# Stefo01/multigrid_prj

Measured on AMD Instinct MI355X. Metric: V-cycles/sec (3D Poisson 513^3 V(2,2)) + finest-grid smoother GB/s vs HBM roofline, higher is better.
Workload: dtype f64; 1 GPU; 3D Poisson 513^3 nodes (nominal 512^3), 6-level V(2,2), jacobi omega=6/7, full-weighting, coarse 17^3 iterated to rel. residual 0.1, f64; parallelism=single GPU, first_gathered_level=6

## Files before the change

__graft_entry__.py:

```python
import os
import subprocess
import sys

ROOT = os.path.dirname(os.path.abspath(__file__))
if ROOT not in sys.path:
    sys.path.insert(0, ROOT)


def build() -> None:
    from multigrid_prj_amd import build as b
    from multigrid_prj_amd import capi
    path = b.build(force=True, verbose=True)
    lib = capi.load(build_if_missing=False)
    missing = [s for s in capi.EXPORTS if not hasattr(lib, s)]
    assert not missing, missing
    subprocess.run(["make", "-C", os.path.join(ROOT, "oracle"), "-B", "_build/liboracle.so"], check=True)
    subprocess.run(["make", "-C", os.path.join(ROOT, "oracle"), "ref"], check=True)
    b.build_cli()
    build_pairbench()
    print("built", path)


def build_pairbench() -> str:
    from concurrent.futures import ThreadPoolExecutor
    csrc = os.path.join(ROOT, "multigrid_prj_amd", "csrc")
    out = os.path.join(ROOT, "tools", "pairbench")
    srcs = [os.path.join(ROOT, "tools", "pairbench.hip")] + [os.path.join(csrc, f) for f in
            ("mg_jacobi_fast.hip", "mg_pair_wide.hip", "mg_rr_wide.hip", "mg_transfer_fast.hip")]
    deps = srcs + [os.path.join(csrc, f) for f in ("mg_kernels.h", "mg_geom.h", "mg_device.h", "mg_switches.h", "mg_switches.def")]
    if os.path.exists(out) and all(os.path.getmtime(out) >= os.path.getmtime(f) for f in deps):
        return out
    objdir = os.path.join(ROOT, "multigrid_prj_amd", "lib", "obj")
    os.makedirs(objdir, exist_ok=True)
    flags = ["-O3", "--offload-arch=gfx950", "-ffp-contract=off", "-std=c++17", "-I" + os.path.join(ROOT, "include")]

    def cc(src):
        obj = os.path.join(objdir, "pb_" + os.path.basename(src) + ".o")
        subprocess.run(["/opt/rocm/bin/hipcc", *flags, "-c", src, "-o", obj], check=True)
        return obj

    with ThreadPoolExecutor(max_workers=5) as ex:
        objs = list(ex.map(cc, srcs))
    subprocess.run(["/opt/rocm/bin/hipcc", "--offload-arch=gfx950", *objs, "-o", out], check=True)
    return out


def smoke() -> None:
    import numpy as np
    from multigrid_prj_amd import capi
    from oracle import pyoracle as po

    assert capi.device_count() > 0, "smoke() needs a GPU"
    kw = dict(dim=2, n=65, levels=3, alpha=1.0, length=10.0, smoother=capi.SMOOTH_JACOBI)
    b = po.fill_rhs_2d(65, 10.0, 1)
    with capi.Solver(capi.make_desc(**kw)) as s:
        s.set_rhs(b)
        hist, _ = s.solve(1e-11, 50)
        o = po.Solver(po.make_desc(**kw)); o.set_rhs(b)
        href, _ = o.solve(1e-11, 50)
        assert len(hist) == len(href), (len(hist), len(href))
        np.testing.assert_allclose(hist, href, rtol=2e-3)
        np.testing.assert_allclose(s.get_solution(), o.get_solution(), rtol=1e-7, atol=1e-9)
    kw = dict(dim=3, n=65, levels=3, length=1.0, alpha=1.0, cycle=capi.CYCLE_V, smoother=capi.SMOOTH_JACOBI,
              omega=6 / 7, nu_pre=2, nu_post=2, coarse_mode=capi.COARSE_FIXED, coarse_maxit=20, outer_pre_gs=0)
    b = po.fill_rhs_3d(65, 1.0, 1.0, 1)
    with capi.Solver(capi.make_desc(**kw)) as s:
        s.set_rhs(b); s.cycle(); s.cycle()
        o = po.Solver(po.make_desc(**kw)); o.set_rhs(b); o.cycle(); o.cycle()
        assert np.array_equal(s.get_solution(), o.get_solution())
    print("smoke ok: 2-D sawtooth history", hist[-1], "3-D V-cycle bit-exact")


if __name__ == "__main__":
    build() if (len(sys.argv) < 2 or sys.argv[1] == "build") else smoke()
```

multigrid_prj_amd/csrc/mg_pair_wide.hip:

```cpp
#include "mg_kernels.h"
#include "mg_device.h"

#include <algorithm>
#include <cmath>

namespace mg {
namespace {

__device__ __forceinline__ float lane_bcast(float v, int l) { return __int_as_float(__builtin_amdgcn_readlane(__float_as_int(v), l)); }
__device__ __forceinline__ double lane_bcast(double v, int l)
{
    const int lo = __builtin_amdgcn_readlane(__double2loint(v), l), hi = __builtin_amdgcn_readlane(__double2hiint(v), l);
    return __hiloint2double(hi, lo);
}

template <typename T, int TPR, int G, bool DAMPED, bool CORR, bool ZEROU, bool RB = false, bool NORM = false>
__global__ __launch_bounds__(TPR * G) void k_pairw(Geom g, Coef<T> c, T omega, const T *__restrict__ u_,
                                                   const T *__restrict__ rhs_, T *__restrict__ out_, int nby, int zc,
                                                   const T *__restrict__ coarse, Geom gc, int dup_planes,
                                                   double *__restrict__ partials)
{
    constexpr int V = Vec16<T>::n, CV = V / 2, NR = CV + 1;
    constexpr int R = 2, NROW = G * R, S = NROW - 2;
    constexpr int LP = TPR * V + 2 * V;
    typedef T vec __attribute__((ext_vector_type(V)));
    static_assert(G >= 2 && (TPR % 64) == 0, "row-wide wave teams, at least two groups");
    __shared__ __align__(16) T su[ZEROU ? 1 : 2][ZEROU ? 1 : NROW + 2][ZEROU ? V : LP];
    __shared__ __align__(16) T sv[2][NROW][LP];
    __shared__ double snorm[NORM ? TPR * G / 64 : 1];

    const int t = threadIdx.x, lane = t & 63;
    const int grp = __builtin_amdgcn_readfirstlane(t / TPR);
    const int xt = t - grp * TPR;
    const int x0 = V * xt;
    const bool tail = (xt == TPR - 1);
    const bool tailwave = (xt >> 6) == (TPR >> 6) - 1;
    const int i0 = grp * R;
    const bool lo_grp = (grp == 0), hi_grp = (grp == G - 1);
    double nsq = 0.;
    const long long per_copy = (long long)nby * g.nz, total = (dup_planes > 0 ? 2 : 1) * per_copy;
    const int nwg = (int)gridDim.x, wper = nwg >> 3;
    const int wi = xcd_block(blockIdx.x, wper);
    const int nbz = zc > 0 ? (g.nz + zc - 1) / zc : 0;
    const long long items = (dup_planes > 0 ? 2 : 1) * (long long)nby * nbz;
    long long w0 = zc > 0 ? wi : total * wi / nwg;
    const long long w1 = zc > 0 ? items : total * (wi + 1) / nwg;
    while (w0 < w1) {
    bool second;
    int by, z0, z1;
    if (zc > 0) {
        const long long per = (long long)nby * nbz;
        second = w0 >= per;
        const long long wr = w0 - (second ? per : 0);
        const int bz = (int)(wr / nby);
        by = (int)(wr - (long long)bz * nby);
        z0 = bz * zc; z1 = min(z0 + zc, g.nz);
        w0 += nwg;
    } else {
        second = w0 >= per_copy;
        const long long wr = w0 - (second ? per_copy : 0);
        by = (int)(wr / g.nz);
        z0 = (int)(wr - (long long)by * g.nz); z1 = (int)min((long long)g.nz, z0 + (w1 - w0));
        w0 += z1 - z0;
    }
    const long long dup_off = second ? (long long)dup_planes * g.plane : 0;
    const T *__restrict__ u = u_ + dup_off;
    const T *__restrict__ rhs = rhs_ + dup_off;
    T *__restrict__ out = out_ + dup_off;
    const int Y0 = by * S;

    long long urow[R];
    bool ybnd[R], outrow[R];
#pragma unroll
    for (int r = 0; r < R; r++) {
        const int y = Y0 + i0 + r, yc = min(y, g.ny - 1);
        ybnd[r] = (yc == 0) || (yc == g.ny - 1);
        urow[r] = (long long)yc * g.pitch;
        const int i = i0 + r;
        outrow[r] = (i >= 1 || by == 0) && (i <= NROW - 2) && (y < g.ny);
    }
    const int hy = lo_grp ? max(Y0 - 1, 0) : min(Y0 + NROW, g.ny - 1);
    const long long hrow = (long long)hy * g.pitch;
    const int hs = lo_grp ? 0 : NROW + 1;

    const int zhalo = (g.gnz != g.nz) ? 2 : 1;
    const int gzo = g.gz0 + (second ? dup_planes : 0), gzn = g.gnz;
    auto plane_of = [&](int p) { return (long long)min(max(p, -zhalo), g.nz - 1 + zhalo) * g.plane; };

    const T hf = (T)0.5;
    typedef T cwide __attribute__((ext_vector_type(NR <= 2 ? 2 : 4), aligned(CV * sizeof(T))));
    int crow[3] = {0, 0, 0};
    const int ic0 = CV * xt;
    if (CORR) {
        const int A = (Y0 + i0) >> 1;
        crow[0] = min(max(A - 1, 0), gc.ny - 1) * gc.pitch;
        crow[1] = min(A, gc.ny - 1) * gc.pitch;
        crow[2] = min(A + 1, gc.ny - 1) * gc.pitch;
    }
    auto cplane = [&](int P, int up1) {
        const int kc = ((gzo + P + up1) >> 1) - gc.gz0;
        return coarse + (long long)min(max(kc, -zhalo), gc.nz - 1 + zhalo) * gc.plane;
    };
    auto load_crow = [&](const T *base, int j, T (&d)[NR]) {
        const cwide w = *(const cwide *)((base + crow[j]) + ic0);
#pragma unroll
        for (int m = 0; m < NR; m++) d[m] = w[m];
    };
    auto raw = [&](int P, T (&Ra)[3][NR], T (&Rb)[3][NR]) {
        const T *c0 = cplane(P, 0);
        const bool odd = ((gzo + P) & 1) != 0;
        const T *c1 = cplane(P, 1);
#pragma unroll
        for (int j = 0; j < 3; j++) {
            if (j == 0 && !lo_grp) {
#pragma unroll
                for (int m = 0; m < NR; m++) { Ra[j][m] = 0; Rb[j][m] = 0; }
                continue;
            }
            load_crow(c0, j, Ra[j]);
            if (odd) load_crow(c1, j, Rb[j]);
            else {
#pragma unroll
                for (int m = 0; m < NR; m++) Rb[j][m] = 0;
            }
        }
    };
    auto zfin = [&](int P, const T (&Ra)[3][NR], const T (&Rb)[3][NR], T (&Z)[3][NR]) {
        const int gP = gzo + P;
        const bool in = (gP >= 0) && (gP < gzn), odd = (gP & 1) != 0;
#pragma unroll
        for (int j = 0; j < 3; j++) {
#pragma unroll
            for (int m = 0; m < NR; m++) {
                const T z = odd ? hf * (Ra[j][m] + Rb[j][m]) : Ra[j][m];
                Z[j][m] = in ? z : (T)0;
            }
        }
    };
    auto pe_vec = [&](const T (&Yr)[NR]) {
        vec w;
#pragma unroll
        for (int mm = 0; mm < CV; mm++) {
            w[2 * mm] = Yr[mm];
            w[2 * mm + 1] = hf * (Yr[mm] + Yr[mm + 1]);
        }
        return w;
    };
    auto add_vec = [&](vec a, vec w) {
        vec o;
#pragma unroll
        for (int e = 0; e < V; e++) o[e] = a[e] + w[e];
        return o;
    };
    auto correct = [&](const T (&Z)[3][NR], vec (&w)[R], T (&tl)[R], vec &h, T &htl, bool with_halo) {
        T Yodd[NR];
#pragma unroll
        for (int m = 0; m < NR; m++) Yodd[m] = hf * (Z[1][m] + Z[2][m]);
        w[0] = add_vec(w[0], pe_vec(Z[1]));
        w[1] = add_vec(w[1], pe_vec(Yodd));
        tl[0] = tl[0] + Z[1][CV];
        tl[1] = tl[1] + Yodd[CV];
        if (with_halo) {
            if (lo_grp) {
                T Yh[NR];
#pragma unroll
                for (int m = 0; m < NR; m++) Yh[m] = hf * (Z[0][m] + Z[1][m]);
                h = add_vec(h, pe_vec(Yh));
                htl = htl + Yh[CV];
            } else if (hi_grp) {
                h = add_vec(h, pe_vec(Z[2]));
                htl = htl + Z[2][CV];
            }
        }
    };

    auto update = [&](const vec &zm, const vec &cc, const vec &zp, const vec &ym, const vec &yp, T xm, T xp,
                      const vec &bb, bool rb) {
        T num[V], quo[V];
        vec res;
#pragma unroll
        for (int e = 0; e < V; e++) {
            const T left = (e == 0) ? xm : cc[e > 0 ? e - 1 : 0];
            const T right = (e == V - 1) ? xp : cc[e < V - 1 ? e + 1 : 0];
            T sum = 0;
            sum += c.cz * zm[e];
            sum += c.cy * ym[e];
            sum += c.cx * left;
            sum += c.cx * right;
            sum += c.cy * yp[e];
            sum += c.cz * zp[e];
            num[e] = bb[e] - sum;
        }
        if constexpr (sizeof(T) == 8) div_cd_n_wave<T, V>(num, quo, c);
        else div_cd_n<T, V>(num, quo, c);
#pragma unroll
        for (int e = 0; e < V; e++) {
            T jac = quo[e];
            if (DAMPED) jac = cc[e] + omega * (jac - cc[e]);
            res[e] = (rb || (x0 + e == 0)) ? bb[e] : jac;
        }
        return res;
    };

    auto resid_sq = [&](const vec &zm, const vec &cc, const vec &zp, const vec &ym, const vec &yp, T xm, T xp,
                        const vec &bb, bool rb) {
        double sq = 0.;
#pragma unroll
        for (int e = 0; e < V; e++) {
            const T left = (e == 0) ? xm : cc[e > 0 ? e - 1 : 0];
            const T right = (e == V - 1) ? xp : cc[e < V - 1 ? e + 1 : 0];
            T sum = 0;
            sum += c.cz * zm[e];
            sum += c.cy * ym[e];
            sum += c.cx * left;
            sum += c.cd * cc[e];
            sum += c.cx * right;
            sum += c.cy * yp[e];
            sum += c.cz * zp[e];
            if (rb || (x0 + e == 0)) sum = (T)1 * cc[e];
            const T res = bb[e] - sum;
            sq += (double)res * (double)res;
        }
        return sq;
    };
    vec um[R], uc[R], up[R], vm[R], vc[R], bq[R];
    {
        T ter[R];
        vec hh = (vec)(0);
        T hter = 0;
#pragma unroll
        for (int r = 0; r < R; r++) {
            um[r] = ZEROU ? (vec)(0) : *(const vec *)((u + (plane_of(z0 - 2) + urow[r])) + x0);
            uc[r] = ZEROU ? (vec)(0) : *(const vec *)((u + (plane_of(z0 - 1) + urow[r])) + x0);
            ter[r] = 0;
            if (tail && !ZEROU) ter[r] = (u + (plane_of(z0 - 1) + urow[r]))[x0 + V];
        }
        if (!ZEROU && (lo_grp || hi_grp)) {
            hh = *(const vec *)((u + (plane_of(z0 - 1) + hrow)) + x0);
            if (tail) hter = (u + (plane_of(z0 - 1) + hrow))[x0 + V];
        }
        if (CORR) {
            T Ra[3][NR], Rb[3][NR], Z[3][NR];
            T dummy_t[R] = {0, 0};
            vec dummy_h = (vec)(0);
            T dummy_ht = 0;
            raw(z0 - 2, Ra, Rb); zfin(z0 - 2, Ra, Rb, Z);
            correct(Z, um, dummy_t, dummy_h, dummy_ht, false);
            raw(z0 - 1, Ra, Rb); zfin(z0 - 1, Ra, Rb, Z);
            correct(Z, uc, ter, hh, hter, true);
        }
        if constexpr (!ZEROU) {
            const int sl = (z0 - 1) & 1;
#pragma unroll
            for (int r = 0; r < R; r++) {
                *(vec *)&su[sl][1 + i0 + r][V + x0] = uc[r];
                if (tail) su[sl][1 + i0 + r][V + x0 + V] = ter[r];
                if (xt == 0) { su[0][1 + i0 + r][V - 1] = 0; su[1][1 + i0 + r][V - 1] = 0; }
            }
            if (lo_grp || hi_grp) {
                *(vec *)&su[sl][hs][V + x0] = hh;
                if (tail) su[sl][hs][V + x0 + V] = hter;
                if (xt == 0) { su[0][hs][V - 1] = 0; su[1][hs][V - 1] = 0; }
            }
        }
        if (xt == 0) {
#pragma unroll
            for (int r = 0; r < R; r++) { sv[0][i0 + r][V - 1] = 0; sv[1][i0 + r][V - 1] = 0; }
        }
    }
    __syncthreads();
#pragma unroll
    for (int r = 0; r < R; r++) { vm[r] = (vec)(0); vc[r] = (vec)(0); bq[r] = (vec)(0); }

    vec nu[R], nb[R], nh = (vec)(0);
    T nter[R], nvt[R], nhter = 0;
    auto fetch_u = [&](int pu1) {
        const long long pn = plane_of(pu1);
#pragma unroll
        for (int r = 0; r < R; r++) nu[r] = ZEROU ? (vec)(0) : *(const vec *)((u + (pn + urow[r])) + x0);
        if (!ZEROU && (lo_grp || hi_grp)) nh = *(const vec *)((u + (pn + hrow)) + x0);
#pragma unroll
        for (int r = 0; r < R; r++) nter[r] = 0;
        if (tail) {
#pragma unroll
            for (int r = 0; r < R; r++) if (!ZEROU) nter[r] = (u + (pn + urow[r]))[x0 + V];
            if (!ZEROU && (lo_grp || hi_grp)) nhter = (u + (pn + hrow))[x0 + V];
        }
    };
    auto fetch_b = [&](int pb) {
        const long long po = plane_of(pb);
#pragma unroll
        for (int r = 0; r < R; r++) nb[r] = *(const vec *)((rhs + (po + urow[r])) + x0);
#pragma unroll
        for (int r = 0; r < R; r++) nvt[r] = 0;
        if (tail) {
#pragma unroll
            for (int r = 0; r < R; r++) nvt[r] = (rhs + (po + urow[r]))[x0 + V];
        }
    };
    auto fetch = [&](int pu1, int pb) { fetch_u(pu1); fetch_b(pb); };
    fetch(z0, z0 - 1);

    for (int p = z0 - 1; p <= z1; p++) {
        vec b[R], hn = nh;
        T vtail[R], ter_n[R], hter_n = nhter;
#pragma unroll
        for (int r = 0; r < R; r++) { up[r] = nu[r]; b[r] = nb[r]; ter_n[r] = nter[r]; vtail[r] = nvt[r]; }
        T Ra[3][NR], Rb[3][NR];
        if (CORR) raw(p + 1, Ra, Rb);
        if (CORR) {
            T Z[3][NR];
            zfin(p + 1, Ra, Rb, Z);
            correct(Z, up, ter_n, hn, hter_n, true);
        }
        if constexpr (!ZEROU) {
            const int sn = (p + 1) & 1;
#pragma unroll
            for (int r = 0; r < R; r++) *(vec *)&su[sn][1 + i0 + r][V + x0] = up[r];
            if (lo_grp || hi_grp) *(vec *)&su[sn][hs][V + x0] = hn;
        }
        if (tail) {
#pragma unroll
            for (int r = 0; r < R; r++) {
                if constexpr (!ZEROU) su[(p + 1) & 1][1 + i0 + r][V + x0 + V] = ter_n[r];
                sv[p & 1][i0 + r][V + x0 + V] = vtail[r];
            }
            if constexpr (!ZEROU) {
                if (lo_grp || hi_grp) su[(p + 1) & 1][hs][V + x0 + V] = hter_n;
            }
        }
        vec v[R];
        {
            const int sc = p & 1;
            const bool zbp = (gzo + p == 0) || (gzo + p == gzn - 1);
#pragma unroll
            for (int r = 0; r < R; r++) {
                T xm = 0, xp = 0;
                vec yo = (vec)(0);
                if constexpr (!ZEROU) {
                    xm = su[sc][1 + i0 + r][V + x0 - 1];
                    xp = su[sc][1 + i0 + r][V + x0 + V];
                    yo = *(const vec *)&su[sc][(r == 0) ? i0 : i0 + 3][V + x0];
                }
                const vec ym = (r == 0) ? yo : uc[0];
                const vec yp = (r == 0) ? uc[1] : yo;
                v[r] = update(um[r], uc[r], up[r], ym, yp, xm, xp, b[r], zbp || ybnd[r]);
                if (NORM && outrow[r] && p >= z0 && p < z1) {
                    nsq += resid_sq(um[r], uc[r], up[r], ym, yp, xm, xp, b[r], zbp || ybnd[r]);
                    if (tail) {
                        const T rt = vtail[r] - (T)1 * xp;
                        nsq += (double)rt * (double)rt;
                    }
                }
                if (RB) {
#pragma unroll
                    for (int e = 0; e < V; e++)
                        if (((x0 + e + Y0 + i0 + r + gzo + p) & 1) != 0) v[r][e] = uc[r][e];
                }
                *(vec *)&sv[sc][i0 + r][V + x0] = v[r];
            }
        }
        constexpr bool LATE_B = !CORR && !ZEROU;
        fetch_u(p + 2);
        if (!LATE_B) fetch_b(p + 1);
        const int q = p - 1;
        if (q >= z0 && q < z1) {
            const bool zbq = (gzo + q == 0) || (gzo + q == gzn - 1);
            const int sl = q & 1;
            const long long qo = (long long)q * g.plane;
#pragma unroll
            for (int r = 0; r < R; r++) {
                if (outrow[r]) {
                    const int i = i0 + r;
                    const T xm = sv[sl][i][V + x0 - 1], xp = sv[sl][i][V + x0 + V];
                    const vec yo = *(const vec *)&sv[sl][(r == 0) ? max(i - 1, 0) : i + 1][V + x0];
                    const vec ym = (r == 0) ? yo : vc[0];
                    const vec yp = (r == 0) ? vc[1] : yo;
                    vec res = update(vm[r], vc[r], v[r], ym, yp, xm, xp, bq[r], zbq || ybnd[r]);
                    if (RB) {
#pragma unroll
                        for (int e = 0; e < V; e++)
                            if (((x0 + e + Y0 + i + gzo + q) & 1) == 0) res[e] = vc[r][e];
                    }
                    __builtin_nontemporal_store(res, (vec *)((out + (qo + urow[r])) + x0));
                    constexpr int LINE = 128 / (int)sizeof(T), TLN = LINE / V;
                    if (tailwave && lane >= 64 - TLN) {
                        const int j = lane - (64 - TLN);
                        const int xs = g.nx - 1 + V * j;
                        const int line_end = ((g.nx - 1) / LINE + 1) * LINE;
                        if (xs < line_end) {
                            const long long rb0 = qo + urow[r];
                            vec tv = (vec)(0);
                            if (j == 0) tv[0] = sv[sl][i][V + TPR * V];
                            __builtin_nontemporal_store(tv, (vec *)(out + rb0 + xs));
                        }
                    }
                }
            }
        }
        if (LATE_B) fetch_b(p + 1);
        __syncthreads();
#pragma unroll
        for (int r = 0; r < R; r++) { um[r] = uc[r]; uc[r] = up[r]; vm[r] = vc[r]; vc[r] = v[r]; bq[r] = b[r]; }
    }
    }
    if (NORM) {
#pragma unroll
        for (int off = 32; off > 0; off >>= 1) nsq += __shfl_down(nsq, off, 64);
        if (lane == 0) snorm[t >> 6] = nsq;
        __syncthreads();
        if (t == 0) {
            double tot = 0.;
            for (int w = 0; w < TPR * G / 64; w++) tot += snorm[w];
            partials[blockIdx.x] = tot;
        }
    }
}

static ChunkPlan wide_plan(const Geom &g, int nby, int ncopy)
{
    return chunk_plan(g.nz, nby, ncopy, cu_count_x8(), 3, std::max(1, g.nz / 4), 1, 3.5, switches().pw_mode, switches().pw_zc);
}

int g_wide_mode = -1;

}

void set_pair_wide(int mode) { g_wide_mode = mode; }

template <typename T>
bool pair_wide_ok(const Geom &g)
{
    constexpr int V = Vec16<T>::n;
    if (g_wide_mode == 0 || (g_wide_mode < 0 && !switches().pair_wide) || g.dim != 3 || (g.nx - 1) % V != 0) return false;
    const int tpr = (g.nx - 1) / V;
    if (tpr != 128 && tpr != 256) return false;
    constexpr int min_rows = 200;
    return g.ny >= min_rows && g.nz >= 8;
}

template <typename T>
int launch_pair_wide(hipStream_t s, const Geom &g, const Geom &gc, const Coef<T> &c, T omega, const T *u, const T *coarse,
                     const T *rhs, T *out, bool zero_u, bool rb, int dup, double *d_partials)
{
    constexpr int V = Vec16<T>::n;
    const int tpr = (g.nx - 1) / V;
    const int G = 1024 / tpr, S = 2 * G - 2;
    const int nby = (g.ny - 1 + S - 1) / S;
    const int ncopy = dup > 0 ? 2 : 1;
    const ChunkPlan plan = wide_plan(g, nby, ncopy);
    const int grid = plan.grid, zc = plan.zc;
    const bool damped = (omega != (T)1) && !rb;
#define MG_PW(TPR, GG, D, C, Z, RBB) \
    hipLaunchKernelGGL((k_pairw<T, TPR, GG, D, C, Z, RBB>), dim3(grid), dim3(TPR * GG), 0, s, g, c, omega, u, rhs, out, nby, zc, coarse, gc, dup, (double *)nullptr)
#define MG_PWN(TPR, GG, D) \
    hipLaunchKernelGGL((k_pairw<T, TPR, GG, D, false, false, false, true>), dim3(grid), dim3(TPR * GG), 0, s, g, c, omega, u, rhs, out, nby, zc, coarse, gc, dup, d_partials)
#define MG_PWNRB(TPR, GG) \
    hipLaunchKernelGGL((k_pairw<T, TPR, GG, false, false, false, true, true>), dim3(grid), dim3(TPR * GG), 0, s, g, c, omega, u, rhs, out, nby, zc, coarse, gc, dup, d_partials)
    const bool norm = d_partials && !coarse && !zero_u;
#define MG_PW_SHAPE(TPR, GG) \
    do { \
        if (norm) { if (rb) MG_PWNRB(TPR, GG); else if (damped) MG_PWN(TPR, GG, true); else MG_PWN(TPR, GG, false); } \
        else if (rb) { if (coarse) MG_PW(TPR, GG, false, true, false, true); else if (zero_u) MG_PW(TPR, GG, false, false, true, true); else MG_PW(TPR, GG, false, false, false, true); } \
        else if (coarse) { if (damped) MG_PW(TPR, GG, true, true, false, false); else MG_PW(TPR, GG, false, true, false, false); } \
        else if (zero_u) { if (damped) MG_PW(TPR, GG, true, false, true, false); else MG_PW(TPR, GG, false, false, true, false); } \
        else { if (damped) MG_PW(TPR, GG, true, false, false, false); else MG_PW(TPR, GG, false, false, false, false); } \
    } while (0)
    (void)G;
    if (tpr == 256) MG_PW_SHAPE(256, 4);
    else MG_PW_SHAPE(128, 8);
#undef MG_PW_SHAPE
#undef MG_PW
#undef MG_PWN
#undef MG_PWNRB
    return norm ? grid : 0;
}

template bool pair_wide_ok<double>(const Geom &);
template bool pair_wide_ok<float>(const Geom &);
template int launch_pair_wide<double>(hipStream_t, const Geom &, const Geom &, const Coef<double> &, double, const double *, const double *, const double *, double *, bool, bool, int, double *);
template int launch_pair_wide<float>(hipStream_t, const Geom &, const Geom &, const Coef<float> &, float, const float *, const float *, const float *, float *, bool, bool, int, double *);

}
```

Baseline: 443.5 V-cycles/s.

## Reuse coarse-plane rows across z-steps and spill CORR rolling state to LDS

In the correction variant of the wide pair kernel, the coarse-grid rows are now carried across iterations in CA/CB registers. Each coarse plane is loaded once and shifted on odd planes, instead of re-reading both coarse planes every z step. The rolling um/uc/vm/vc register state is reloaded from the shared-memory planes rather than kept in registers, which is meant to lower register pressure. A foldcheck tool is also added to the build. This trades more LDS reads for fewer global coarse loads and VGPRs, with a risk of subtle indexing errors.

```diff
diff --git a/__graft_entry__.py b/__graft_entry__.py
--- a/__graft_entry__.py
+++ b/__graft_entry__.py
@@ -25,10 +25,12 @@
     from concurrent.futures import ThreadPoolExecutor
     csrc = os.path.join(ROOT, "multigrid_prj_amd", "csrc")
     out = os.path.join(ROOT, "tools", "pairbench")
-    srcs = [os.path.join(ROOT, "tools", "pairbench.hip")] + [os.path.join(csrc, f) for f in
-            ("mg_jacobi_fast.hip", "mg_pair_wide.hip", "mg_rr_wide.hip", "mg_transfer_fast.hip")]
+    tools = [os.path.join(ROOT, "tools", f) for f in ("pairbench.hip", "foldcheck.hip")]
+    kernels = [os.path.join(csrc, f) for f in ("mg_jacobi_fast.hip", "mg_pair_wide.hip", "mg_rr_wide.hip", "mg_transfer_fast.hip")]
+    srcs = tools + kernels
     deps = srcs + [os.path.join(csrc, f) for f in ("mg_kernels.h", "mg_geom.h", "mg_device.h", "mg_switches.h", "mg_switches.def")]
-    if os.path.exists(out) and all(os.path.getmtime(out) >= os.path.getmtime(f) for f in deps):
+    outs = [t[:-len(".hip")] for t in tools]
+    if all(os.path.exists(o) and all(os.path.getmtime(o) >= os.path.getmtime(f) for f in deps) for o in outs):
         return out
     objdir = os.path.join(ROOT, "multigrid_prj_amd", "lib", "obj")
     os.makedirs(objdir, exist_ok=True)
@@ -39,9 +41,10 @@
         subprocess.run(["/opt/rocm/bin/hipcc", *flags, "-c", src, "-o", obj], check=True)
         return obj
 
-    with ThreadPoolExecutor(max_workers=5) as ex:
+    with ThreadPoolExecutor(max_workers=6) as ex:
         objs = list(ex.map(cc, srcs))
-    subprocess.run(["/opt/rocm/bin/hipcc", "--offload-arch=gfx950", *objs, "-o", out], check=True)
+    for o, tool_obj in zip(outs, objs):
+        subprocess.run(["/opt/rocm/bin/hipcc", "--offload-arch=gfx950", tool_obj, *objs[len(tools):], "-o", o], check=True)
     return out
 
 
diff --git a/multigrid_prj_amd/csrc/mg_pair_wide.hip b/multigrid_prj_amd/csrc/mg_pair_wide.hip
--- a/multigrid_prj_amd/csrc/mg_pair_wide.hip
+++ b/multigrid_prj_amd/csrc/mg_pair_wide.hip
@@ -125,6 +125,13 @@
             }
         }
     };
+    auto load_rows = [&](const T *base, T (&Rw)[3][NR]) {
+#pragma unroll
+        for (int j = 0; j < 3; j++) {
+            if (j == 0 && !lo_grp) continue;
+            load_crow(base, j, Rw[j]);
+        }
+    };
     auto zfin = [&](int P, const T (&Ra)[3][NR], const T (&Rb)[3][NR], T (&Z)[3][NR]) {
         const int gP = gzo + P;
         const bool in = (gP >= 0) && (gP < gzn), odd = (gP & 1) != 0;
@@ -254,6 +261,7 @@
 #pragma unroll
             for (int r = 0; r < R; r++) {
                 *(vec *)&su[sl][1 + i0 + r][V + x0] = uc[r];
+                if constexpr (CORR) *(vec *)&su[sl ^ 1][1 + i0 + r][V + x0] = um[r];
                 if (tail) su[sl][1 + i0 + r][V + x0 + V] = ter[r];
                 if (xt == 0) { su[0][1 + i0 + r][V - 1] = 0; su[1][1 + i0 + r][V - 1] = 0; }
             }
@@ -300,17 +308,40 @@
     };
     auto fetch = [&](int pu1, int pb) { fetch_u(pu1); fetch_b(pb); };
     fetch(z0, z0 - 1);
+    T CA[3][NR], CB[3][NR];
+#pragma unroll
+    for (int j = 0; j < 3; j++) {
+#pragma unroll
+        for (int m = 0; m < NR; m++) { CA[j][m] = 0; CB[j][m] = 0; }
+    }
+    if constexpr (CORR) {
+        load_rows(cplane(z0, 0), CA);
+        if (((gzo + z0) & 1) != 0) load_rows(cplane(z0, 1), CB);
+    }
 
     for (int p = z0 - 1; p <= z1; p++) {
         vec b[R], hn = nh;
         T vtail[R], ter_n[R], hter_n = nhter;
+        if constexpr (CORR) {
+#pragma unroll
+            for (int r = 0; r < R; r++) {
+                um[r] = *(const vec *)&su[(p + 1) & 1][1 + i0 + r][V + x0];
+                uc[r] = *(const vec *)&su[p & 1][1 + i0 + r][V + x0];
+            }
+        }
 #pragma unroll
         for (int r = 0; r < R; r++) { up[r] = nu[r]; b[r] = nb[r]; ter_n[r] = nter[r]; vtail[r] = nvt[r]; }
-        T Ra[3][NR], Rb[3][NR];
-        if (CORR) raw(p + 1, Ra, Rb);
-        if (CORR) {
+        const bool codd = ((gzo + p + 1) & 1) != 0;
+        if constexpr (CORR) {
             T Z[3][NR];
-            zfin(p + 1, Ra, Rb, Z);
+            zfin(p + 1, CA, CB, Z);
+            if (codd) {
+#pragma unroll
+                for (int j = 0; j < 3; j++) {
+#pragma unroll
+                    for (int m = 0; m < NR; m++) CA[j][m] = CB[j][m];
+                }
+            }
             correct(Z, up, ter_n, hn, hter_n, true);
         }
         if constexpr (!ZEROU) {
@@ -357,17 +388,25 @@
                     for (int e = 0; e < V; e++)
                         if (((x0 + e + Y0 + i0 + r + gzo + p) & 1) != 0) v[r][e] = uc[r][e];
                 }
+                if constexpr (CORR) vm[r] = *(const vec *)&sv[sc][i0 + r][V + x0];
                 *(vec *)&sv[sc][i0 + r][V + x0] = v[r];
             }
         }
         constexpr bool LATE_B = !CORR && !ZEROU;
         fetch_u(p + 2);
         if (!LATE_B) fetch_b(p + 1);
+        if constexpr (CORR) {
+            if (!codd && p < z1) load_rows(cplane(p + 2, 1), CB);
+        }
         const int q = p - 1;
         if (q >= z0 && q < z1) {
             const bool zbq = (gzo + q == 0) || (gzo + q == gzn - 1);
             const int sl = q & 1;
             const long long qo = (long long)q * g.plane;
+            if constexpr (CORR) {
+#pragma unroll
+                for (int r = 0; r < R; r++) vc[r] = *(const vec *)&sv[sl][i0 + r][V + x0];
+            }
 #pragma unroll
             for (int r = 0; r < R; r++) {
                 if (outrow[r]) {
@@ -401,7 +440,10 @@
         if (LATE_B) fetch_b(p + 1);
         __syncthreads();
 #pragma unroll
-        for (int r = 0; r < R; r++) { um[r] = uc[r]; uc[r] = up[r]; vm[r] = vc[r]; vc[r] = v[r]; bq[r] = b[r]; }
+        for (int r = 0; r < R; r++) {
+            if constexpr (!CORR) { um[r] = uc[r]; uc[r] = up[r]; vm[r] = vc[r]; vc[r] = v[r]; }
+            bq[r] = b[r];
+        }
     }
     }
     if (NORM) {
```

After: 448.6 V-cycles/s, median of 6. 1.01x the previous value.
